# ERGO-Code/ipx

Measured on AMD Instinct MI355X. Metric: kkt_solves_per_sec, higher is better.
Workload: dtype f64

## Files before the change

ipx_amd/csrc/internal.hpp:

```cpp
#pragma once

#include <hip/hip_runtime.h>

#include <cstdint>
#include <cstdio>
#include <cstdlib>
#include <algorithm>
#include <cstring>
#include <memory>
#include <stdexcept>
#include <string>
#include <type_traits>
#include <vector>

#include "../../include/ipx_kkt_hip.h"

namespace ipxk {

struct Error : std::runtime_error {
    int code;
    Error(int c, const std::string& what) : std::runtime_error(what), code(c) {}
};

void set_last_error(const std::string& msg);
// ... 69 lines not shown
constexpr int kLongSeg = 2048;
constexpr int kMaxWorkgroups = 1024;
constexpr int kMaxPartials = 2048;
constexpr int kMaxRT = 8;

struct GatherView {
    int nrows, ncols;
    int P, G, RT, Q;
    int RWrows;
    const int* step_ptr;
    const int* wg_chunk_ptr;
    const int* chunk_start;
    const int* chunk_info;
    const int* chunk_step;
    const unsigned char* counts;
    const int* idx;
    const double* val;
    const unsigned char* row_long;
    int nseg;
    const int* seg_p0;
    const int* seg_p1;
    const int* lidx;
    const double* lval;
    int nlong;
    const int* long_row;
    const int* long_slot;
    double* long_partials;
    unsigned long long* stamps;
    int masked;
};

constexpr int kSlicedRows = 1024;
constexpr int kSlicedMaxTile = 7680;

struct SlicedView {
    int nrows, nrows_pad, nslices, nrb;
    int R;
    const unsigned* tile_ptr;
    const unsigned char* cnt;
    const int* idx;
    const double* val;
    double* partial;
    const unsigned char* row_long;
    int masked;
};

struct SlicedMatrix {
    bool built = false;
    int nslices = 0, nrb = 0, nrows_pad = 0, max_tile = 0, R = kSlicedRows;
    double dominant_fraction = 1.0;
    DevBuf<unsigned> tile_ptr;
    DevBuf<unsigned char> cnt;
    DevBuf<int> idx;
    DevBuf<double> val, partial;
};

constexpr int kSortedThreads = 256;
constexpr int kSortedMaxSub = 8192;
constexpr int kSortedOffBits = 18;
struct SortedView {
    int nrows, nrows_pad, nslices, nsub, nrb, RB, slice_elems;
    const int* xmin;
    const unsigned char* row_long;
    const unsigned* sub_ptr;
    const unsigned char* cnt;
    const unsigned* pack;
    const double* val;
    double* partial;
};
struct SortedMatrix {
    bool built = false;
    int nslices = 0, nsub = 0, nrb = 0, RB = 0, nrows_pad = 0, max_sub = 0, slice_elems = 0;
    DevBuf<unsigned> sub_ptr, pack;
    DevBuf<unsigned char> cnt;
    DevBuf<double> val, partial;
    bool fused = false;
    DevBuf<int> xmin;
};

constexpr int kAccThreads = 512;
constexpr int kAccPerThread = 4;
constexpr int kAccBatch = kAccThreads * kAccPerThread;
constexpr int kAccMaxRows = 16384;
struct AccView {
    int nrows, nrows_pad, nslices, nrb, RB, slice_elems;
    const int* xmin;
    const unsigned* tile_batch;
    const unsigned* bptr;
    const unsigned* pack;
    const double* val;
    double* partial;
};
struct AccMatrix {
    bool built = false;
    int nslices = 0, nrb = 0, RB = 0, nrows_pad = 0, slice_elems = 0;
    int64_t nbatches = 0, deferred = 0;
    DevBuf<unsigned> tile_batch, bptr, pack;
    DevBuf<double> val, partial;
    bool fused = false;
    DevBuf<int> xmin;
};

struct LayoutScratch;

struct GatherMatrix {
    int nrows = 0, ncols = 0;
    int64_t nnz = 0;
    int P = 1, G = 1, RT = 1, Q = 1, RWrows = kBlock;
    DevBuf<int> step_ptr, idx, wg_chunk_ptr, chunk_start, chunk_info, chunk_step;
    DevBuf<unsigned char> counts, row_long;
    DevBuf<double> val;
    int nseg = 0, nlong = 0;
    DevBuf<int> seg_p0, seg_p1, lidx, long_row, long_slot;
    DevBuf<double> lval, long_partials;
    DevBuf<unsigned long long> stamps;
    int tune_level = 2;
    bool keep_plain = false;
    std::vector<int> h_plain_ptr;
    DevBuf<int> plain_idx;
    DevBuf<double> plain_val;

    void build(int64_t nrows_, int64_t ncols_, const ipxint* hptr, const ipxint* hidx,
               const double* hval, hipStream_t s);
    bool build_device(LayoutScratch& S, int64_t nrows_, int64_t ncols_, int64_t nnz_, const int* dptr, const int* didx,
                      const double* dval, hipStream_t s);
    bool build_device_local(LayoutScratch& S, int64_t nrows_, int64_t ncols_, int64_t nnz_, const int* dptr, const int* didx,
                            const double* dval, double share, hipStream_t s);
    void set_geometry(int64_t nrows_, int64_t ncols_);
    SlicedMatrix sliced;
    bool use_sliced = false;
    SortedMatrix sorted;
    bool use_sorted = false;
    void build_sorted(const ipxint* hptr, const ipxint* hidx, const double* hval, hipStream_t s);
    AccMatrix acc;
    bool use_acc = false;
    float tuned_us_acc = 0.f;
    void build_acc(const ipxint* hptr, const ipxint* hidx, const double* hval, hipStream_t s);
    void build_acc_fused(const ipxint* hptr, const ipxint* hidx, const double* hval, hipStream_t s);
    AccMatrix accf;
    bool use_acc_fused = false;
    float tuned_us_acc_fused = 0.f;
    AccView acc_fused_view() const;
    AccView acc_view() const;
    const int* csr_ptr = nullptr;
    const int* csr_idx = nullptr;
    const double* csr_val = nullptr;
    bool use_plain = false;
    float tuned_us_plain = 0.f;
    int plain_grid() const { return (int)std::min<int64_t>(kMaxPartials, std::max<int64_t>(1, ((int64_t)nrows * 8 + kBlock - 1) / kBlock)); }
    void build_sorted_fused(const ipxint* hptr, const ipxint* hidx, const double* hval, hipStream_t s);
    bool use_sorted_fused = false;
    float tuned_us_sorted_fused = 0.f;
    int sorted_fused_grid() const {
        static const int cap = [] { const char* e = getenv("IPXK_SF_GRID"); return e && atoi(e) > 0 ? std::min(atoi(e), kMaxPartials) : kMaxPartials; }();
        return std::min(sorted.nrb, cap);
    }
    SortedView sorted_view() const;
    float tuned_us_phased = 0.f, tuned_us_sliced = 0.f, tuned_us_fused = 0.f, tuned_us_sorted = 0.f;
    void build_sliced(const ipxint* hptr, const ipxint* hidx, const double* hval, hipStream_t s, int ns_request);
    SlicedView sliced_view(int which = 0) const;
    int fused_grid() const { return std::min(sliced.nrb, kMaxPartials); }
    int combine_grid() const { return (int)std::min<int64_t>(1024, std::max<int64_t>(1, ((int64_t)nrows + kBlock - 1) / kBlock)); }

    GatherView view(bool masked = false) const;
    int grid() const { return G; }
    DevBuf<double> valM, lvalM;
// ... 40 lines not shown
```

ipx_amd/csrc/layout_device.hip:

```cpp
#include <rocprim/device/device_radix_sort.hpp>
#include <rocprim/device/device_scan.hpp>

#include <chrono>
#include <memory>

#include "context.hpp"

namespace ipxk {

namespace {

using u64 = unsigned long long;
#define IPXK_GS(i, n) for (int64_t i = (int64_t)blockIdx.x * blockDim.x + threadIdx.x; i < (n); i += (int64_t)gridDim.x * blockDim.x)

int gridn(int64_t n) { return (int)std::min<int64_t>(8192, std::max<int64_t>(1, (n + kBlock - 1) / kBlock)); }
int bits_for(u64 maxval) { int b = 1; while (b < 64 && (maxval >> b) != 0) b++; return b; }

__global__ void narrow_kernel(int64_t nz, const ipxint* __restrict__ in, int* __restrict__ out, int limit, int* bad) {
    IPXK_GS(p, nz) {
        const ipxint v = in[p];
        if (v < 0 || v >= limit) *bad = 1;
        out[p] = (int)v;
    }
}
__global__ void rowof_kernel(int nrows, const int* __restrict__ ptr, int* __restrict__ rowof, unsigned* __restrict__ pos) {
    IPXK_GS(r, nrows)
        for (int p = ptr[r]; p < ptr[r + 1]; p++) { rowof[p] = (int)r; if (pos) pos[p] = (unsigned)p; }
}
__global__ void gather_transposed_kernel(int64_t nz, const unsigned* __restrict__ perm, const int* __restrict__ colof,
                                         const double* __restrict__ Ax, int* __restrict__ Ti, double* __restrict__ Tx) {
    IPXK_GS(t, nz) {
        const unsigned p = perm[t];
        Ti[t] = colof[p];
        Tx[t] = Ax[p];
    }
}
template <class K>
__global__ void lower_bounds_kernel(int64_t count, int64_t nz, const K* __restrict__ sorted, u64 stride, int shift, unsigned* __restrict__ out) {
    IPXK_GS(t, count) {
        const u64 want = (u64)t * stride;
        int64_t lo = 0, hi = nz;
        while (lo < hi) { const int64_t mid = (lo + hi) >> 1; if (((u64)sorted[mid] >> shift) < want) lo = mid + 1; else hi = mid; }
        out[t] = (unsigned)lo;
    }
}
__global__ void row_pointers_kernel(int64_t m, int64_t nz, const unsigned* __restrict__ sorted_rows, int* __restrict__ Tp) {
    IPXK_GS(i, m + 1) {
        int64_t lo = 0, hi = nz;
        while (lo < hi) { const int64_t mid = (lo + hi) >> 1; if (sorted_rows[mid] < (unsigned)i) lo = mid + 1; else hi = mid; }
        Tp[i] = (int)lo;
    }
}
__global__ void max_len_kernel(int nrows, const int* __restrict__ ptr, int* out) {
    int best = 0;
    IPXK_GS(r, nrows) best = max(best, ptr[r + 1] - ptr[r]);
#pragma unroll
    for (int d = 32; d >= 1; d >>= 1) best = max(best, __shfl_xor(best, d, 64));
    if ((threadIdx.x & 63) == 0 && best > 0) atomicMax(out, best);
}
__global__ void row_extent_kernel(int n, const int* __restrict__ rows, const int* __restrict__ ptr, int* __restrict__ ext) {
    IPXK_GS(l, n) { ext[2 * l] = ptr[rows[l]]; ext[2 * l + 1] = ptr[rows[l] + 1]; }
}
__global__ void sliced_keys_kernel(int nrows, const int* __restrict__ ptr, const int* __restrict__ idx, int R, int ns, int slice,
                                   unsigned* __restrict__ key, unsigned* __restrict__ pos) {
    IPXK_GS(r, nrows) {
        const unsigned base = (unsigned)(r / R) * (unsigned)ns, rr = (unsigned)(r % R);
        for (int p = ptr[r]; p < ptr[r + 1]; p++) {
            key[p] = (base + (unsigned)(idx[p] / slice)) * (unsigned)R + rr;
            pos[p] = (unsigned)p;
        }
    }
}
__global__ void sorted_keys1_kernel(int nrows, const int* __restrict__ ptr, const int* __restrict__ idx, int RB, int ns, int nsub, int slice,
                                    int half, unsigned* __restrict__ key, unsigned* __restrict__ pos) {
    IPXK_GS(r, nrows) {
        const unsigned tile0 = (unsigned)(r / RB) * (unsigned)ns, rr = (unsigned)(r % RB);
        for (int p = ptr[r]; p < ptr[r + 1]; p++) {
            const int sl = idx[p] / slice, off = idx[p] - sl * slice;
            const unsigned sub = (tile0 + (unsigned)sl) * (unsigned)nsub + (unsigned)min(off / half, nsub - 1);
            key[p] = sub * (unsigned)RB + rr;
            pos[p] = (unsigned)p;
        }
// ... 490 lines not shown
        out.tile_ptr.ensure((size_t)ntiles + 1);
        hipLaunchKernelGGL(lower_bounds_kernel<unsigned>, dim3(gridn(ntiles + 1)), dim3(kBlock), 0, s, ntiles + 1, nnz, S.k2.get(), (u64)R, 0,
                           out.tile_ptr.get());
        IPXK_HIP(hipMemsetAsync(S.stats.get(), 0, 8 * sizeof(int), s));
        hipLaunchKernelGGL(tile_stats_kernel, dim3(gridn(nrb)), dim3(kBlock), 0, s, nrb, ns, out.tile_ptr.get(), S.stats.get());
        IPXK_HIP(hipMemcpyAsync(h, S.stats.get(), sizeof h, hipMemcpyDeviceToHost, s));
        IPXK_HIP(hipStreamSynchronize(s));
        if (h[0] <= kSlicedMaxTile) break;
    }
    u64 dom = 0;
    memcpy(&dom, h + 2, sizeof dom);
    out.dominant_fraction = (double)(int64_t)dom / (double)nnz;
    const size_t nslots = (size_t)ntiles * R;
    out.cnt.ensure(nslots); out.idx.ensure(nz); out.val.ensure(nz);
    IPXK_HIP(hipMemsetAsync(out.cnt.get(), 0, nslots, s));
    IPXK_HIP(hipMemsetAsync(S.stats.get(), 0, 8 * sizeof(int), s));
    hipLaunchKernelGGL(run_counts_kernel, dim3(gridn(nnz)), dim3(kBlock), 0, s, nnz, S.k2.get(), out.cnt.get(), S.stats.get());
    hipLaunchKernelGGL(gather_entries_kernel, dim3(gridn(nnz)), dim3(kBlock), 0, s, nnz, S.v2.get(), didx, dval, out.idx.get(), out.val.get());
    int over = 0;
    IPXK_HIP(hipMemcpyAsync(&over, S.stats.get(), sizeof(int), hipMemcpyDeviceToHost, s));
    IPXK_HIP(hipStreamSynchronize(s));
    IPXK_HIP(hipGetLastError());
    if (over) { out = SlicedMatrix(); return false; }
    out.R = R; out.nslices = ns; out.nrb = nrb; out.nrows_pad = nrb * R; out.max_tile = h[0];
    out.partial.resize(ns > 1 ? (size_t)ns * out.nrows_pad : 1);
    out.built = true;
    return true;
}

bool device_build_sorted(LayoutScratch& S, SortedMatrix& out, const SlicedMatrix& sliced, int nrows, int ncols, int64_t nnz, const int* dptr,
                         const int* didx, const double* dval, hipStream_t s) {
    out = SortedMatrix();
    if (!sliced.built || sliced.nslices < 2 || nnz == 0) return false;
    const int ns = sliced.nslices;
    const int64_t slice = (((int64_t)ncols + ns - 1) / ns + 15) / 16 * 16;
    if (slice > (int64_t(1) << kSortedOffBits)) return false;
    static const int nsub_env = [] { const char* e = getenv("IPXK_SORTED_NSUB"); return e && atoi(e) > 0 ? std::min(atoi(e), 16) : 2; }();
    const int nsub = nsub_env;
    const int64_t half = (slice / nsub + 15) / 16 * 16;
    const size_t nz = (size_t)nnz;
    S.k1.ensure(nz); S.k2.ensure(nz); S.v1.ensure(nz); S.v2.ensure(nz); S.v3.ensure(nz); S.v4.ensure(nz); S.q1.ensure(nz); S.q2.ensure(nz);
    S.stats.ensure(8);
    int RB = 32 * kSortedThreads, nrb = 0, max_sub = 0;
    int64_t nsubs = 0;
    for (;; RB /= 2) {
        if (RB < 4 * kSortedThreads) return false;
        nrb = (nrows + RB - 1) / RB;
        nsubs = (int64_t)nrb * ns * nsub;
        if ((u64)nsubs * (u64)RB >= (u64(1) << 32)) return false;
        hipLaunchKernelGGL(sorted_keys1_kernel, dim3(gridn(nrows)), dim3(kBlock), 0, s, nrows, dptr, didx, RB, ns, nsub, (int)slice, (int)half,
                           S.k1.get(), S.v1.get());
        sort_pairs<unsigned>(S.T, S.k1.get(), S.k2.get(), S.v1.get(), S.v2.get(), nz, bits_for((u64)nsubs * (u64)RB - 1), s);
        out.sub_ptr.ensure((size_t)nsubs + 1);
        hipLaunchKernelGGL(lower_bounds_kernel<unsigned>, dim3(gridn(nsubs + 1)), dim3(kBlock), 0, s, nsubs + 1, nnz, S.k2.get(), (u64)RB, 0,
                           out.sub_ptr.get());
        IPXK_HIP(hipMemsetAsync(S.stats.get(), 0, 8 * sizeof(int), s));
        hipLaunchKernelGGL(max_range_kernel, dim3(gridn(nsubs)), dim3(kBlock), 0, s, nsubs, out.sub_ptr.get(), S.stats.get());
        IPXK_HIP(hipMemcpyAsync(&max_sub, S.stats.get(), sizeof(int), hipMemcpyDeviceToHost, s));
        IPXK_HIP(hipStreamSynchronize(s));
        if (max_sub <= kSortedMaxSub) break;
    }
    const size_t nslots = (size_t)nsubs * RB;
    out.cnt.ensure(nslots); out.pack.ensure(nz); out.val.ensure(nz);
    IPXK_HIP(hipMemsetAsync(out.cnt.get(), 0, nslots, s));
    IPXK_HIP(hipMemsetAsync(S.stats.get(), 0, 8 * sizeof(int), s));
    hipLaunchKernelGGL(run_counts_kernel, dim3(gridn(nnz)), dim3(kBlock), 0, s, nnz, S.k2.get(), out.cnt.get(), S.stats.get());
    hipLaunchKernelGGL(sorted_keys2_kernel, dim3(gridn(nnz)), dim3(kBlock), 0, s, nnz, S.k2.get(), S.v2.get(), didx, RB, ns, nsub, (int)slice,
                       S.q1.get(), S.v3.get());
    sort_pairs<u64>(S.T, S.q1.get(), S.q2.get(), S.v3.get(), S.v4.get(), nz, kSortedOffBits + bits_for((u64)nsubs - 1), s);
    hipLaunchKernelGGL(sorted_fill_kernel, dim3(gridn(nnz)), dim3(kBlock), 0, s, nnz, S.q2.get(), S.v4.get(), S.v2.get(), out.sub_ptr.get(), dval,
                       out.pack.get(), out.val.get());
    int over = 0;
    IPXK_HIP(hipMemcpyAsync(&over, S.stats.get(), sizeof(int), hipMemcpyDeviceToHost, s));
    IPXK_HIP(hipStreamSynchronize(s));
    IPXK_HIP(hipGetLastError());
    if (over) { out = SortedMatrix(); return false; }
    out.nslices = ns; out.nsub = nsub; out.nrb = nrb; out.RB = RB; out.nrows_pad = nrb * RB;
    out.max_sub = max_sub; out.slice_elems = (int)slice;
    out.partial.resize((size_t)ns * out.nrows_pad);
    out.built = true;
    return true;
}

int acc_rows_per_block(int nrows, int ns) {
    static const int cap = [] { const char* e = getenv("IPXK_ACC_ROWS"); return e && atoi(e) >= 1024 ? std::min(atoi(e), kAccMaxRows) : kAccMaxRows; }();
    int RB = cap;
    while (RB > 1024 && ((int64_t)nrows + RB - 1) / RB * (int64_t)ns < 256) RB /= 2;
    return RB;
}

bool device_build_acc(LayoutScratch& S, AccMatrix& out, const SlicedMatrix& sliced, int nrows, int ncols, int64_t nnz, const int* dptr,
                      const int* didx, const double* dval, hipStream_t s) {
    out = AccMatrix();
    if (!sliced.built || sliced.nslices < 2 || nnz == 0) return false;
    const int ns = sliced.nslices;
    const int64_t slice = (((int64_t)ncols + ns - 1) / ns + 15) / 16 * 16;
    if (slice > (int64_t(1) << kSortedOffBits)) return false;
    const int RB = acc_rows_per_block(nrows, ns);
    const int nrb = (nrows + RB - 1) / RB;
    const int64_t ntiles = (int64_t)nrb * ns;
    const size_t nz = (size_t)nnz;
    S.q1.ensure(nz); S.q2.ensure(nz); S.v1.ensure(nz); S.v2.ensure(nz); S.v3.ensure(nz); S.v4.ensure(nz); S.k1.ensure(nz); S.k2.ensure(nz);
    S.stats.ensure(8);
    DevBuf<int> rowof(nz);
    DevBuf<unsigned> tile_ptr((size_t)ntiles + 1), nbatch((size_t)ntiles + 1), bstart(nz);
    hipLaunchKernelGGL(acc_keys_kernel, dim3(gridn(nrows)), dim3(kBlock), 0, s, nrows, dptr, didx, RB, ns, (int)slice, S.q1.get(), S.v1.get(), rowof.get());
    sort_pairs<u64>(S.T, S.q1.get(), S.q2.get(), S.v1.get(), S.v2.get(), nz, kSortedOffBits + bits_for((u64)std::max<int64_t>(ntiles, 2) - 1), s);
    hipLaunchKernelGGL(lower_bounds_kernel<u64>, dim3(gridn(ntiles + 1)), dim3(kBlock), 0, s, ntiles + 1, nnz, S.q2.get(), (u64)1, kSortedOffBits,
                       tile_ptr.get());
    unsigned* word = S.k1.get();
    hipLaunchKernelGGL(acc_words_kernel, dim3(gridn(nnz)), dim3(kBlock), 0, s, nnz, S.q2.get(), S.v2.get(), rowof.get(), RB, word);
    IPXK_HIP(hipMemsetAsync(S.stats.get(), 0, 8 * sizeof(int), s));
    const size_t lds = (size_t)RB * 2 * sizeof(unsigned);
    IPXK_HIP(hipFuncSetAttribute(reinterpret_cast<const void*>(acc_batch_kernel), hipFuncAttributeMaxDynamicSharedMemorySize,
                                 (int)(kAccMaxRows * 2 * sizeof(unsigned))));
    hipLaunchKernelGGL(acc_batch_kernel, dim3((unsigned)ntiles), dim3(64), lds, s, RB, tile_ptr.get(), word, S.k2.get(), S.v3.get(), S.v4.get(),
                       bstart.get(), nbatch.get(), reinterpret_cast<u64*>(S.stats.get()));
    out.tile_batch.ensure((size_t)ntiles + 1);
    hipLaunchKernelGGL(scan_u32_kernel, dim3(1), dim3(1024), 0, s, (int)ntiles, nbatch.get(), out.tile_batch.get());
    unsigned nb_total = 0;
    u64 ndef = 0;
    IPXK_HIP(hipMemcpyAsync(&nb_total, out.tile_batch.get() + ntiles, sizeof(unsigned), hipMemcpyDeviceToHost, s));
    IPXK_HIP(hipMemcpyAsync(&ndef, S.stats.get(), sizeof(u64), hipMemcpyDeviceToHost, s));
    IPXK_HIP(hipStreamSynchronize(s));
    out.bptr.ensure((size_t)nb_total + 1); out.pack.ensure(nz); out.val.ensure(nz);
    hipLaunchKernelGGL(acc_bptr_kernel, dim3((unsigned)ntiles), dim3(64), 0, s, (int)ntiles, tile_ptr.get(), out.tile_batch.get(), bstart.get(),
                       (unsigned)nnz, out.bptr.get());
    hipLaunchKernelGGL(acc_scatter_kernel, dim3(gridn(nnz)), dim3(kBlock), 0, s, nnz, S.k2.get(), word, S.v2.get(), dval, out.pack.get(),
                       out.val.get());
    IPXK_HIP(hipStreamSynchronize(s));
    IPXK_HIP(hipGetLastError());
    out.nslices = ns; out.nrb = nrb; out.RB = RB; out.nrows_pad = nrb * RB; out.slice_elems = (int)slice;
    out.nbatches = nb_total; out.deferred = (int64_t)ndef;
    out.partial.resize((size_t)ns * out.nrows_pad);
    out.built = true;
    return true;
}

bool device_build_sorted_fused(LayoutScratch& S, SortedMatrix& out, int nrows, int ncols, int64_t nnz, const int* dptr, const int* didx,
                               const double* dval, hipStream_t s) {
    out = SortedMatrix();
    if (nrows == 0 || nnz == 0 || ncols == 0) return false;
    static const int cap = [] { const char* e = getenv("IPXK_SF_MAXSUB"); return e && atoi(e) >= 256 ? std::min(atoi(e), kSortedMaxSub) : kSortedMaxSub; }();
    const size_t nz = (size_t)nnz;
    S.q1.ensure(nz); S.q2.ensure(nz); S.v1.ensure(nz); S.v2.ensure(nz); S.stats.ensure(8);
    DevBuf<int> lo, hi;
    int RB = 32 * kSortedThreads, nrb = 0, h[4] = {0, 0, 0, 0};
    for (;; RB /= 2) {
        if (RB < kSortedThreads) return false;
        nrb = (nrows + RB - 1) / RB;
        if (RB > kSortedThreads && nrb < 1024) continue;
        lo.ensure((size_t)nrb); hi.ensure((size_t)nrb);
        out.cnt.ensure((size_t)nrb * RB);
        IPXK_HIP(hipMemsetAsync(lo.get(), 0x7f, (size_t)nrb * sizeof(int), s));
        IPXK_HIP(hipMemsetAsync(hi.get(), 0xff, (size_t)nrb * sizeof(int), s));
        IPXK_HIP(hipMemsetAsync(out.cnt.get(), 0, (size_t)nrb * RB, s));
        IPXK_HIP(hipMemsetAsync(S.stats.get(), 0, 8 * sizeof(int), s));
        hipLaunchKernelGGL(tile_window_kernel, dim3(gridn(nrows)), dim3(kBlock), 0, s, nrows, dptr, didx, RB, lo.get(), hi.get(), out.cnt.get(), S.stats.get() + 2);
        hipLaunchKernelGGL(tile_window_stats_kernel, dim3(gridn(nrb)), dim3(kBlock), 0, s, nrb, nrows, RB, dptr, lo.get(), hi.get(), S.stats.get());
        IPXK_HIP(hipMemcpyAsync(h, S.stats.get(), sizeof h, hipMemcpyDeviceToHost, s));
        IPXK_HIP(hipStreamSynchronize(s));
        if (h[2]) { out = SortedMatrix(); return false; }
        if (h[1] <= cap) break;
    }
    if (h[0] >= (1 << kSortedOffBits)) { out = SortedMatrix(); return false; }
    hipLaunchKernelGGL(fused_keys_kernel, dim3(gridn(nrows)), dim3(kBlock), 0, s, nrows, dptr, didx, RB, lo.get(), S.q1.get(), S.v1.get(), (int*)nullptr);
    sort_pairs<u64>(S.T, S.q1.get(), S.q2.get(), S.v1.get(), S.v2.get(), nz, kSortedOffBits + bits_for((u64)std::max(nrb, 2) - 1), s);
    out.sub_ptr.ensure((size_t)nrb + 1); out.pack.ensure(nz); out.val.ensure(nz); out.xmin.ensure((size_t)nrb);
// ... 314 lines not shown
```

ipx_amd/csrc/nmatrix.hip:

```cpp
#include <rocprim/device/device_radix_sort.hpp>
#include <rocprim/device/device_scan.hpp>

#include "context.hpp"
#include "spmv_kernels.hpp"
#include "trisolve.hpp"

namespace ipxk {

namespace {

using u64 = unsigned long long;
constexpr int kTileShift = 42, kRowShift = 32;
#define IPXK_GS(i, n) for (int64_t i = (int64_t)blockIdx.x * blockDim.x + threadIdx.x; i < (n); i += (int64_t)gridDim.x * blockDim.x)

int gridn(int64_t n) { return (int)std::min<int64_t>(4096, std::max<int64_t>(1, (n + kBlock - 1) / kBlock)); }

__global__ void nm_keep_kernel(int n, const double* __restrict__ W, const int* __restrict__ Ap, int* __restrict__ keep, int* __restrict__ len) {
    IPXK_GS(j, n) {
        const int k = W[j] != 0.0 ? 1 : 0;
        keep[j] = k;
        len[j] = k ? Ap[j + 1] - Ap[j] : 0;
    }
}
__global__ void nm_colof_kernel(int n, const int* __restrict__ keep, const int* __restrict__ newidx, int* __restrict__ colof,
// ... 221 lines not shown
        const int nN = last[0] + last[1];
        const int64_t nzN = (int64_t)last[2] + last[3];
        if (nN < 1 || nzN < 1) return false;
        N.nN = nN;
        N.colof.ensure((size_t)nN);
        hipLaunchKernelGGL(nm_colof_kernel, dim3(gridn(n)), dim3(kBlock), 0, s, n, N.keep.get(), N.newidx.get(), N.colof.get(), N.newidx.get());
        N.keys.ensure((size_t)c->nnz); N.keys2.ensure((size_t)c->nnz);
        int64_t slice1 = 0, slice2 = 0;
        const int ns1 = slices_for(m, &slice1), ns2 = slices_for(nN, &slice2);
        N.P1 = SlicedMatrix(); N.P2 = SlicedMatrix();
        bool ok = false;
        for (int R = kSlicedRows; R >= kBlock && !ok; R /= 2) {
            hipLaunchKernelGGL(nm_keys_p1_kernel, dim3(gridn(n)), dim3(kBlock), 0, s, n, c->pl_Ap.get(), c->pl_Ai.get(), N.newidx.get(), N.off.get(), R,
                               ns1, (int)slice1, N.keys.get());
            sort_u64(N.T, N.keys.get(), N.keys2.get(), (size_t)nzN, s);
            ok = finish_layout(N, N.P1, nN, R, ns1, nzN, N.keys2.get(), c->pl_Ai.get(), c->pl_Ax.get(), nullptr, s);
        }
        if (!ok) return false;
        ok = false;
        for (int R = kSlicedRows; R >= kBlock && !ok; R /= 2) {
            hipLaunchKernelGGL(nm_keys_p2_kernel, dim3(gridn(m)), dim3(kBlock), 0, s, m, c->pl_Tp.get(), c->pl_Ti.get(), N.newidx.get(), R, ns2, (int)slice2,
                               N.keys.get());
            sort_u64(N.T, N.keys.get(), N.keys2.get(), (size_t)c->nnz, s);
            ok = finish_layout(N, N.P2, m, R, ns2, nzN, N.keys2.get(), c->pl_Ti.get(), c->pl_Tx.get(), N.newidx.get(), s);
        }
        if (!ok) return false;
        N.A1 = AccMatrix(); N.A2 = AccMatrix();
        if (!(getenv("IPXK_SPMV_ACC") && getenv("IPXK_SPMV_ACC")[0] == '0') && ns1 > 1 && ns2 > 1) {
            std::unique_ptr<LayoutScratch, void (*)(LayoutScratch*)> LS(new_layout_scratch(), free_layout_scratch);
            const size_t nzn = (size_t)nzN;
            N.cptr.ensure((size_t)std::max(nN, m) + 1); N.cidx.ensure(nzn); N.cval.ensure(nzn);
            hipLaunchKernelGGL(nm_csr1_kernel, dim3(gridn(nN)), dim3(kBlock), 0, s, nN, nzN, N.colof.get(), N.off.get(), c->pl_Ap.get(), c->pl_Ai.get(),
                               c->pl_Ax.get(), N.cptr.get(), N.cidx.get(), N.cval.get());
            AccMatrix a1, a2;
            const bool ok1 = device_build_acc(*LS, a1, N.P1, nN, m, nzN, N.cptr.get(), N.cidx.get(), N.cval.get(), s);
            N.cnt32.ensure((size_t)m + 1);
            hipLaunchKernelGGL(nm_csr2_count_kernel, dim3(gridn(m)), dim3(kBlock), 0, s, m, c->pl_Tp.get(), c->pl_Ti.get(), N.newidx.get(), N.cnt32.get());
            scan_int(N.T, N.cnt32.get(), N.cptr.get(), (size_t)m, s);
            hipLaunchKernelGGL(nm_csr2_fill_kernel, dim3(gridn(m)), dim3(kBlock), 0, s, m, nzN, c->pl_Tp.get(), c->pl_Ti.get(), c->pl_Tx.get(),
                               N.newidx.get(), N.cptr.get(), N.cidx.get(), N.cval.get());
            const bool ok2 = device_build_acc(*LS, a2, N.P2, m, nN, nzN, N.cptr.get(), N.cidx.get(), N.cval.get(), s);
            if (ok1 && ok2) { N.A1 = std::move(a1); N.A2 = std::move(a2); }
        }
        N.wN.ensure((size_t)nN); N.tN.ensure((size_t)nN);
        N.kept_hash = hsh;
        N.keep_built.ensure((size_t)n);
        IPXK_HIP(hipMemcpyAsync(N.keep_built.get(), N.keep.get(), (size_t)n * sizeof(int), hipMemcpyDeviceToDevice, s));
        N.valid = true;
        if (getenv("IPXK_VERBOSE"))
            fprintf(stderr, "ipxk: N built on the device: %d of %d structural columns, %lld entries; N'u tiles %d x %d (rows %d), N t tiles %d x %d (rows %d)\n",
                    nN, n, (long long)nzN, N.P1.nrb, N.P1.nslices, N.P1.R, N.P2.nrb, N.P2.nslices, N.P2.R);
    }
    hipLaunchKernelGGL(nm_weights_kernel, dim3(gridn(N.nN)), dim3(kBlock), 0, s, N.nN, N.colof.get(), W, N.wN.get());
    IPXK_HIP(hipGetLastError());
    return true;
}

void nmatrix_invalidate(Context* c) { if (c->nmat) c->nmat->valid = false; }

static SlicedView view_of(const SlicedMatrix& P, int nrows) {
    SlicedView V;
    V.nrows = nrows; V.nrows_pad = P.nrows_pad; V.nslices = P.nslices; V.nrb = P.nrb; V.R = P.R;
    V.tile_ptr = P.tile_ptr.get(); V.cnt = P.cnt.get(); V.idx = P.idx.get(); V.val = P.val.get(); V.partial = P.partial.get();
    V.row_long = nullptr; V.masked = 0;
    return V;
}
template <class Epi>
static void launch_tiles(const SlicedMatrix& P, int nrows, const double* x, const Epi& epi, const int* done, hipStream_t s) {
    const SlicedView V = view_of(P, nrows);
    const size_t lds = (size_t)(P.max_tile + P.max_tile / 32 + 1) * sizeof(double);
    const dim3 grid(V.nrb * V.nslices), block(kBlock);
    if (V.R == kBlock * 4) hipLaunchKernelGGL((spmv_sliced_tile_kernel<Epi, 4, false, false>), grid, block, lds, s, V, x, epi, (double*)nullptr, done);
    else if (V.R == kBlock * 2) hipLaunchKernelGGL((spmv_sliced_tile_kernel<Epi, 2, false, false>), grid, block, lds, s, V, x, epi, (double*)nullptr, done);
    else hipLaunchKernelGGL((spmv_sliced_tile_kernel<Epi, 1, false, false>), grid, block, lds, s, V, x, epi, (double*)nullptr, done);
    const int cg = (int)std::min<int64_t>(1024, std::max<int64_t>(1, ((int64_t)nrows + kBlock - 1) / kBlock));
    hipLaunchKernelGGL(spmv_sliced_combine_kernel<Epi>, dim3(cg), dim3(kBlock), 0, s, V, epi, (double*)nullptr, done);
}

template <class Epi>
static void launch_acc(const AccMatrix& A, const SlicedMatrix& P, int nrows, const double* x, const Epi& epi, const int* done, hipStream_t s) {
    AccView W;
    W.nrows = nrows; W.nrows_pad = A.nrows_pad; W.nslices = A.nslices; W.nrb = A.nrb; W.RB = A.RB; W.slice_elems = A.slice_elems;
    W.tile_batch = A.tile_batch.get(); W.bptr = A.bptr.get(); W.pack = A.pack.get(); W.val = A.val.get(); W.partial = A.partial.get();
    static bool lds_attr_set = false;
    if (!lds_attr_set) {
        IPXK_HIP(hipFuncSetAttribute(reinterpret_cast<const void*>(spmv_acc_tile_kernel<Epi>), hipFuncAttributeMaxDynamicSharedMemorySize,
                                     (int)(kAccMaxRows * sizeof(double))));
        lds_attr_set = true;
    }
    hipLaunchKernelGGL((spmv_acc_tile_kernel<Epi>), dim3(W.nrb * W.nslices), dim3(kAccThreads), (size_t)W.RB * sizeof(double), s, W, x, done);
    SlicedView V = view_of(P, nrows);
    V.nrows_pad = A.nrows_pad; V.partial = A.partial.get();
    const int cg = (int)std::min<int64_t>(1024, std::max<int64_t>(1, ((int64_t)nrows + kBlock - 1) / kBlock));
    hipLaunchKernelGGL(spmv_sliced_combine_kernel<Epi>, dim3(cg), dim3(kBlock), 0, s, V, epi, (double*)nullptr, done);
}

void nmatrix_apply(Context* c, const double* WI, const double* u, double* work, const int* done) {
    NMatrix& N = *c->nmat;
    hipStream_t s = c->stream;
    EpiScale e1{{}, N.wN.get(), N.tN.get()};
    EpiNormalRows e2{{}, WI, u, work};
    if (N.A1.built && N.A2.built) {
        launch_acc(N.A1, N.P1, N.nN, u, e1, done, s);
        launch_acc(N.A2, N.P2, (int)c->m, N.tN.get(), e2, done, s);
        return;
    }
    launch_tiles(N.P1, N.nN, u, e1, done, s);
    launch_tiles(N.P2, (int)c->m, N.tN.get(), e2, done, s);
}

}
```

ipx_amd/csrc/spmv_kernels.hpp:

```cpp
#pragma once

#include "device_utils.hpp"
#include "internal.hpp"

namespace ipxk {

constexpr int kLdsDoubles = kChunkNnz + kChunkNnz / 32;

__device__ __forceinline__ int lds_slot(int q) { return q + (q >> 5); }

struct ProdMul {
    static __device__ __forceinline__ double prod(double xg, double v) { return xg * v; }
};
struct ProdSquareWeighted {
    static __device__ __forceinline__ double prod(double xg, double v) { return (v * xg) * v; }
};

struct EpiScale : ProdMul {
    const double* w; double* out;
    static constexpr bool kNeg = false;
    __device__ __forceinline__ double init(int) const { return 0.0; }
    __device__ __forceinline__ void finish(int r, double acc, double&) const {
        out[r] = w ? acc * w[r] : acc;
    }
// ... 535 lines not shown
            p += cq;
        }
        __syncthreads();
    }
    if (dot_partials) {
        double d = dotpart;
#pragma unroll
        for (int o = 32; o > 0; o >>= 1) d += __shfl_down(d, o, 64);
        if (lane == 0) red[wave] = d;
        __syncthreads();
        if (tid == 0) {
            double t = 0.0;
            for (int w = 0; w < kSortedThreads / 64; w++) t += red[w];
            dot_partials[blockIdx.x] = t;
        }
    }
}

template <class Prod>
__global__ __launch_bounds__(kAccThreads) void spmv_acc_tile_kernel(AccView M, const double* __restrict__ x, const int* done) {
    if (done && *done) return;
    extern __shared__ double ac_sum[];
    constexpr int U = kAccPerThread, T = kAccThreads;
    const int tid = threadIdx.x;
    const int tile = blockIdx.x, s = tile % M.nslices, rb = tile / M.nslices;
    const double* __restrict__ xs = x + (size_t)s * M.slice_elems;
    const unsigned b0 = M.tile_batch[tile];
    const int nb = (int)(M.tile_batch[tile + 1] - b0);
    auto first = [&](int k) -> unsigned { return M.bptr[b0 + min(k, nb)]; };
    constexpr int NE = 6;
    unsigned e[NE];
#pragma unroll
    for (int i = 0; i < NE; i++) e[i] = first(i);
    unsigned pk[3][U];
    double v[3][U], xg[2][U];
    auto stream = [&](unsigned (&pkb)[U], double (&vb)[U], unsigned e0, unsigned e1) {
        const int ne = (int)(e1 - e0);
        if (ne <= 0) return;
#pragma unroll
        for (int u = 0; u < U; u++) {
            const int i = min(u * T + tid, ne - 1);
            pkb[u] = __builtin_nontemporal_load(M.pack + e0 + i);
            vb[u] = __builtin_nontemporal_load(M.val + e0 + i);
        }
    };
    auto gather = [&](double (&xgb)[U], const unsigned (&pkb)[U]) {
#pragma unroll
        for (int u = 0; u < U; u++) xgb[u] = xs[pkb[u] & ((1u << kSortedOffBits) - 1u)];
    };
#pragma unroll
    for (int d = 0; d < 3; d++) {
#pragma unroll
        for (int u = 0; u < U; u++) { pk[d][u] = 0u; v[d][u] = 0.0; }
        stream(pk[d], v[d], e[d], e[d + 1]);
    }
    for (int r = tid; r < M.RB; r += T) ac_sum[r] = 0.0;
    if (nb > 0) gather(xg[0], pk[0]);
    for (int k0 = 0; k0 < nb; k0 += 6) {
#pragma unroll
        for (int d = 0; d < 6; d++) {
            const int k = k0 + d;
            if (k < nb) {
                const int ne = (int)(e[1] - e[0]);
                if (k + 1 < nb) gather(xg[(d + 1) & 1], pk[(d + 1) % 3]);
                const unsigned enew = first(k + NE);
                __syncthreads();
#pragma unroll
                for (int u = 0; u < U; u++)
                    if (u * T + tid < ne)
                        __hip_atomic_fetch_add(ac_sum + (pk[d % 3][u] >> kSortedOffBits), Prod::prod(xg[d & 1][u], v[d % 3][u]), __ATOMIC_RELAXED,
                                               __HIP_MEMORY_SCOPE_WORKGROUP);
                stream(pk[d % 3], v[d % 3], e[3], e[4]);
#pragma unroll
                for (int i = 0; i + 1 < NE; i++) e[i] = e[i + 1];
                e[NE - 1] = enew;
            }
        }
    }
    __syncthreads();
    double* dst = M.partial + (size_t)s * M.nrows_pad + (size_t)rb * M.RB;
    for (int r = 2 * tid; r < M.RB; r += 2 * T) reinterpret_cast<double2*>(dst + r)[0] = make_double2(ac_sum[r], ac_sum[r + 1]);
}

template <class Epi>
__global__ __launch_bounds__(kBlock) void spmv_rowgroup_kernel(int nrows, const int* __restrict__ ptr, const int* __restrict__ idx,
                                                               const double* __restrict__ val, const unsigned char* __restrict__ row_long,
                                                               const double* __restrict__ x, Epi epi, double* dot_partials, const int* done) {
    if (done && *done) return;
    __shared__ double red[kBlock / 64 + 1];
    const int lane8 = threadIdx.x & 7, lane = threadIdx.x & 63, g0 = lane & ~7;
    double dotpart = 0.0;
    const int ngroups = (gridDim.x * kBlock) >> 3;
    for (int r = (blockIdx.x * kBlock + threadIdx.x) >> 3; r < nrows; r += ngroups) {
        const bool live = !(row_long && row_long[r]);
        const int p0 = ptr[r], p1 = live ? ptr[r + 1] : p0;
        double acc = lane8 == 0 ? epi.init(r) : 0.0;
        for (int p = p0; p < p1; p += 8) {
            const int q = p + lane8;
            const double prod = q < p1 ? Epi::prod(x[idx[q]], val[q]) : 0.0;
#pragma unroll
            for (int k = 0; k < 8; k++) {
                const double t = __shfl(prod, g0 + k, 64);
                if (p + k < p1) acc = Epi::kNeg ? acc - t : acc + t;
            }
        }
        if (live && lane8 == 0) epi.finish(r, acc, dotpart);
    }
    if (dot_partials) {
        const double d = block_reduce<SumOp>(dotpart, red);
        if (threadIdx.x == 0) dot_partials[blockIdx.x] = d;
    }
}

template <class Epi>
__global__ __launch_bounds__(kAccThreads) void spmv_acc_fused_kernel(AccView M, const double* __restrict__ x, Epi epi, double* dot_partials,
                                                                     const int* done) {
    if (done && *done) return;
    extern __shared__ double ac_sum[];
    __shared__ double red[kAccThreads / 64];
    constexpr int U = kAccPerThread, T = kAccThreads;
    const int tid = threadIdx.x;
    const int tile = blockIdx.x;
    const double* __restrict__ xs = x + M.xmin[tile];
    const unsigned b0 = M.tile_batch[tile];
    const int nb = (int)(M.tile_batch[tile + 1] - b0);
    auto first = [&](int k) -> unsigned { return M.bptr[b0 + min(k, nb)]; };
    constexpr int NE = 6;
    unsigned e[NE];
#pragma unroll
    for (int i = 0; i < NE; i++) e[i] = first(i);
    unsigned pk[3][U];
    double v[3][U], xg[2][U];
    auto stream = [&](unsigned (&pkb)[U], double (&vb)[U], unsigned e0, unsigned e1) {
        const int ne = (int)(e1 - e0);
        if (ne <= 0) return;
#pragma unroll
        for (int u = 0; u < U; u++) {
            const int i = min(u * T + tid, ne - 1);
            pkb[u] = __builtin_nontemporal_load(M.pack + e0 + i);
            vb[u] = __builtin_nontemporal_load(M.val + e0 + i);
        }
    };
    auto gather = [&](double (&xgb)[U], const unsigned (&pkb)[U]) {
#pragma unroll
        for (int u = 0; u < U; u++) xgb[u] = xs[pkb[u] & ((1u << kSortedOffBits) - 1u)];
    };
#pragma unroll
    for (int d = 0; d < 3; d++) {
#pragma unroll
        for (int u = 0; u < U; u++) { pk[d][u] = 0u; v[d][u] = 0.0; }
        stream(pk[d], v[d], e[d], e[d + 1]);
    }
    const int r0 = tile * M.RB;
    for (int r = tid; r < M.RB; r += T) ac_sum[r] = r0 + r < M.nrows ? epi.init(r0 + r) : 0.0;
    if (nb > 0) gather(xg[0], pk[0]);
    for (int k0 = 0; k0 < nb; k0 += 6) {
#pragma unroll
        for (int d = 0; d < 6; d++) {
            const int k = k0 + d;
            if (k < nb) {
                const int ne = (int)(e[1] - e[0]);
                if (k + 1 < nb) gather(xg[(d + 1) & 1], pk[(d + 1) % 3]);
                const unsigned enew = first(k + NE);
                __syncthreads();
#pragma unroll
                for (int u = 0; u < U; u++)
                    if (u * T + tid < ne) {
                        const double p = Epi::prod(xg[d & 1][u], v[d % 3][u]);
                        __hip_atomic_fetch_add(ac_sum + (pk[d % 3][u] >> kSortedOffBits), Epi::kNeg ? -p : p, __ATOMIC_RELAXED, __HIP_MEMORY_SCOPE_WORKGROUP);
                    }
                stream(pk[d % 3], v[d % 3], e[3], e[4]);
#pragma unroll
                for (int i = 0; i + 1 < NE; i++) e[i] = e[i + 1];
                e[NE - 1] = enew;
            }
        }
    }
    __syncthreads();
    double dotpart = 0.0;
    for (int r = tid; r < M.RB; r += T)
        if (r0 + r < M.nrows) epi.finish(r0 + r, ac_sum[r], dotpart);
    if (dot_partials) {
#pragma unroll
        for (int o = 32; o > 0; o >>= 1) dotpart += __shfl_down(dotpart, o, 64);
        if ((tid & 63) == 0) red[tid >> 6] = dotpart;
        __syncthreads();
        if (tid == 0) {
            double t = 0.0;
            for (int w = 0; w < T / 64; w++) t += red[w];
            dot_partials[tile] = t;
        }
    }
}

template <class Epi>
__global__ __launch_bounds__(kBlock) void spmv_sliced_combine_kernel(SlicedView M, Epi epi, double* dot_partials,
                                                                     const int* done) {
    if (done && *done) return;
    __shared__ double red[kBlock / 64 + 1];
    double dotpart = 0.0;
    for (int r = blockIdx.x * kBlock + threadIdx.x; r < M.nrows; r += gridDim.x * kBlock) {
        if (M.row_long && M.row_long[r]) continue;
        double acc = epi.init(r);
        for (int s = 0; s < M.nslices; s++) {
            const double t = __builtin_nontemporal_load(M.partial + (size_t)s * M.nrows_pad + r);
            acc = Epi::kNeg ? acc - t : acc + t;
        }
        epi.finish(r, acc, dotpart);
    }
    if (dot_partials) {
        const double d = block_reduce<SumOp>(dotpart, red);
        if (threadIdx.x == 0) dot_partials[blockIdx.x] = d;
    }
}

template <class Epi, bool MASKED = false, bool COMPACT = false>
inline void launch_spmv_sliced(const GatherMatrix& M, const double* x, const Epi& epi, double* dot_partials,
                               const int* done, hipStream_t s) {
    static_assert(!(MASKED && COMPACT), "the compacted copy needs no mask");
    if (M.use_acc && !MASKED && !COMPACT) {
        const AccView W = M.acc_view();
        const size_t lds = (size_t)W.RB * sizeof(double);
        static bool lds_attr_set = false;
        if (!lds_attr_set) {
            IPXK_HIP(hipFuncSetAttribute(reinterpret_cast<const void*>(spmv_acc_tile_kernel<Epi>), hipFuncAttributeMaxDynamicSharedMemorySize,
                                         (int)(kAccMaxRows * sizeof(double))));
            lds_attr_set = true;
        }
        hipLaunchKernelGGL((spmv_acc_tile_kernel<Epi>), dim3(W.nrb * W.nslices), dim3(kAccThreads), lds, s, W, x, done);
        SlicedView C = M.sliced_view(0);
        C.nrows_pad = W.nrows_pad; C.partial = W.partial;
        hipLaunchKernelGGL(spmv_sliced_combine_kernel<Epi>, dim3(M.combine_grid()), dim3(kBlock), 0, s, C, epi, dot_partials, done);
        if (M.nlong > 0) {
            const GatherView G = M.view(false);
            hipLaunchKernelGGL(spmv_long_kernel<Epi>, dim3(M.nseg), dim3(kBlock), 0, s, G, x, done);
            hipLaunchKernelGGL(spmv_long_fixup_kernel<Epi>, dim3(1), dim3(kBlock), 0, s, G, epi, dot_partials, M.combine_grid(), done);
        }
        return;
    }
    const SlicedView V = M.sliced_view(COMPACT ? 2 : MASKED ? 1 : 0);
    const size_t lds = (size_t)(M.sliced.max_tile + M.sliced.max_tile / 32 + 1) * sizeof(double);
    const dim3 grid(V.nrb * V.nslices), block(kBlock);
    if (V.nslices == 1) {
        const dim3 fgrid(M.fused_grid());
        if (V.R == kBlock * 4) hipLaunchKernelGGL((spmv_sliced_tile_kernel<Epi, 4, true, MASKED>), fgrid, block, lds, s, V, x, epi, dot_partials, done);
        else if (V.R == kBlock * 2) hipLaunchKernelGGL((spmv_sliced_tile_kernel<Epi, 2, true, MASKED>), fgrid, block, lds, s, V, x, epi, dot_partials, done);
        else hipLaunchKernelGGL((spmv_sliced_tile_kernel<Epi, 1, true, MASKED>), fgrid, block, lds, s, V, x, epi, dot_partials, done);
    } else {
        if (V.R == kBlock * 4) hipLaunchKernelGGL((spmv_sliced_tile_kernel<Epi, 4, false, MASKED>), grid, block, lds, s, V, x, epi, dot_partials, done);
        else if (V.R == kBlock * 2) hipLaunchKernelGGL((spmv_sliced_tile_kernel<Epi, 2, false, MASKED>), grid, block, lds, s, V, x, epi, dot_partials, done);
        else hipLaunchKernelGGL((spmv_sliced_tile_kernel<Epi, 1, false, MASKED>), grid, block, lds, s, V, x, epi, dot_partials, done);
        hipLaunchKernelGGL(spmv_sliced_combine_kernel<Epi>, dim3(M.combine_grid()), dim3(kBlock), 0, s, V, epi,
                           dot_partials, done);
    }
    if (M.nlong > 0) {
        const GatherView G = M.view(MASKED || COMPACT);
        hipLaunchKernelGGL(spmv_long_kernel<Epi>, dim3(M.nseg), block, 0, s, G, x, done);
        hipLaunchKernelGGL(spmv_long_fixup_kernel<Epi>, dim3(1), block, 0, s, G, epi, dot_partials,
                           V.nslices == 1 ? M.fused_grid() : M.combine_grid(), done);
    }
}

template <class Epi, bool MASKED = false>
inline int launch_spmv(const GatherMatrix& M, const double* x, const Epi& epi, double* dot_partials,
                       const int* done, hipStream_t s) {
    if (M.use_acc_fused && !MASKED) {
        const AccView W = M.acc_fused_view();
        static bool lds_attr_set = false;
        if (!lds_attr_set) {
            IPXK_HIP(hipFuncSetAttribute(reinterpret_cast<const void*>(spmv_acc_fused_kernel<Epi>), hipFuncAttributeMaxDynamicSharedMemorySize,
                                         (int)(kAccMaxRows * sizeof(double))));
            lds_attr_set = true;
        }
        hipLaunchKernelGGL((spmv_acc_fused_kernel<Epi>), dim3(W.nrb), dim3(kAccThreads), (size_t)W.RB * sizeof(double), s, W, x, epi, dot_partials, done);
        return dot_partials ? W.nrb : 0;
    }
    if (M.use_plain && !MASKED) {
        const int grid = M.plain_grid();
        hipLaunchKernelGGL(spmv_rowgroup_kernel<Epi>, dim3(grid), dim3(kBlock), 0, s, M.nrows, M.csr_ptr, M.csr_idx, M.csr_val,
                           M.nlong > 0 ? M.row_long.get() : nullptr, x, epi, dot_partials, done);
        if (M.nlong > 0) {
            const GatherView G = M.view(false);
            hipLaunchKernelGGL(spmv_long_kernel<Epi>, dim3(M.nseg), dim3(kBlock), 0, s, G, x, done);
            hipLaunchKernelGGL(spmv_long_fixup_kernel<Epi>, dim3(1), dim3(kBlock), 0, s, G, epi, dot_partials, grid, done);
        }
        return dot_partials ? grid + (M.nlong > 0 ? 1 : 0) : 0;
    }
    if (M.use_sorted_fused && !MASKED) {
        const SortedView W = M.sorted_view();
        const size_t lds = (size_t)(M.sorted.max_sub + M.sorted.max_sub / 32 + 1) * sizeof(double);
        const dim3 grid(M.sorted_fused_grid()), block(kSortedThreads);
        switch (W.RB / kSortedThreads) {
            case 32: hipLaunchKernelGGL((spmv_sorted_fused_kernel<Epi, 32>), grid, block, lds, s, W, x, epi, dot_partials, done); break;
            case 16: hipLaunchKernelGGL((spmv_sorted_fused_kernel<Epi, 16>), grid, block, lds, s, W, x, epi, dot_partials, done); break;
            case 8: hipLaunchKernelGGL((spmv_sorted_fused_kernel<Epi, 8>), grid, block, lds, s, W, x, epi, dot_partials, done); break;
            case 4: hipLaunchKernelGGL((spmv_sorted_fused_kernel<Epi, 4>), grid, block, lds, s, W, x, epi, dot_partials, done); break;
            case 2: hipLaunchKernelGGL((spmv_sorted_fused_kernel<Epi, 2>), grid, block, lds, s, W, x, epi, dot_partials, done); break;
            default: hipLaunchKernelGGL((spmv_sorted_fused_kernel<Epi, 1>), grid, block, lds, s, W, x, epi, dot_partials, done); break;
        }
        if (M.nlong > 0) {
            const GatherView G = M.view(false);
            hipLaunchKernelGGL(spmv_long_kernel<Epi>, dim3(M.nseg), dim3(kBlock), 0, s, G, x, done);
            hipLaunchKernelGGL(spmv_long_fixup_kernel<Epi>, dim3(1), dim3(kBlock), 0, s, G, epi, dot_partials, M.sorted_fused_grid(), done);
        }
        return dot_partials ? M.sorted_fused_grid() + (M.nlong > 0 ? 1 : 0) : 0;
    }
    if (M.use_sliced) {
        if (MASKED && M.compact.valid) launch_spmv_sliced<Epi, false, true>(M, x, epi, dot_partials, done, s);
        else launch_spmv_sliced<Epi, MASKED>(M, x, epi, dot_partials, done, s);
        return dot_partials ? M.num_partials() : 0;
    }
    const GatherView V = M.view(MASKED);
// ... 16 lines not shown
```

Baseline: 55.06.

## Add persistent LDS-accumulator SpMV kernel with tile-balanced row blocking

Adds a persistent-grid version of the LDS-atomic accumulation SpMV. One block per CU walks tiles with a stride, prefetches packed indices and values several batches ahead, and double-buffers the x gathers. When a tile finishes, its LDS row sums are parked in registers and written out a little at a time, so the stores overlap the next tile's work. Row-block size is also chosen so the tile count divides evenly across the persistent grid. The cost is higher register pressure and more complex synchronisation, and the partial layout now assumes RB-strided tiles, so any error in tile ordering or the parked-store logic would corrupt results.

Measured after the change: 57.31, median of 6. 4.1% higher.

```diff
diff --git a/ipx_amd/csrc/internal.hpp b/ipx_amd/csrc/internal.hpp
--- a/ipx_amd/csrc/internal.hpp
+++ b/ipx_amd/csrc/internal.hpp
@@ -175,6 +175,7 @@
 constexpr int kAccPerThread = 4;
 constexpr int kAccBatch = kAccThreads * kAccPerThread;
 constexpr int kAccMaxRows = 16384;
+int acc_persist_grid(int ns);
 struct AccView {
     int nrows, nrows_pad, nslices, nrb, RB, slice_elems;
     const int* xmin;
diff --git a/ipx_amd/csrc/layout_device.hip b/ipx_amd/csrc/layout_device.hip
--- a/ipx_amd/csrc/layout_device.hip
+++ b/ipx_amd/csrc/layout_device.hip
@@ -1,3 +1,4 @@
+#include <numeric>
 #include <rocprim/device/device_radix_sort.hpp>
 #include <rocprim/device/device_scan.hpp>
 
@@ -654,8 +655,29 @@
     return true;
 }
 
+int acc_persist_grid(int ns) {
+    static const int setting = [] { const char* e = getenv("IPXK_ACC_PERSIST"); return e ? std::max(0, atoi(e)) : 1; }();
+    if (setting == 0 || ns < 1) return 0;
+    static int cus[64] = {};
+    int dev = 0;
+    IPXK_HIP(hipGetDevice(&dev));
+    if (dev < 0 || dev >= 64) dev = 0;
+    if (cus[dev] == 0) IPXK_HIP(hipDeviceGetAttribute(&cus[dev], hipDeviceAttributeMultiprocessorCount, dev));
+    const int L = std::lcm(8, ns);
+    const int n = setting > 1 ? std::min(setting, cus[dev]) : cus[dev];
+    return std::max(L, n / L * L);
+}
+
 int acc_rows_per_block(int nrows, int ns) {
-    static const int cap = [] { const char* e = getenv("IPXK_ACC_ROWS"); return e && atoi(e) >= 1024 ? std::min(atoi(e), kAccMaxRows) : kAccMaxRows; }();
+    static const int cap = [] { const char* e = getenv("IPXK_ACC_ROWS"); return e && atoi(e) >= 1024 ? std::min(atoi(e), kAccMaxRows) & ~1 : kAccMaxRows; }();
+    static const bool balance = !(getenv("IPXK_ACC_BALANCE") && getenv("IPXK_ACC_BALANCE")[0] == '0');
+    if (const int G = balance ? acc_persist_grid(ns) : 0) {
+        const int64_t per = G / ns;
+        const int64_t nrb = (((int64_t)nrows + cap - 1) / cap + per - 1) / per * per;
+        int rb = (int)(((int64_t)nrows + nrb - 1) / nrb);
+        rb += rb & 1;
+        if (rb >= 1024 && 8 * (int64_t)rb >= 7 * (int64_t)cap) return rb;
+    }
     int RB = cap;
     while (RB > 1024 && ((int64_t)nrows + RB - 1) / RB * (int64_t)ns < 256) RB /= 2;
     return RB;
diff --git a/ipx_amd/csrc/nmatrix.hip b/ipx_amd/csrc/nmatrix.hip
--- a/ipx_amd/csrc/nmatrix.hip
+++ b/ipx_amd/csrc/nmatrix.hip
@@ -327,13 +327,7 @@
     AccView W;
     W.nrows = nrows; W.nrows_pad = A.nrows_pad; W.nslices = A.nslices; W.nrb = A.nrb; W.RB = A.RB; W.slice_elems = A.slice_elems;
     W.tile_batch = A.tile_batch.get(); W.bptr = A.bptr.get(); W.pack = A.pack.get(); W.val = A.val.get(); W.partial = A.partial.get();
-    static bool lds_attr_set = false;
-    if (!lds_attr_set) {
-        IPXK_HIP(hipFuncSetAttribute(reinterpret_cast<const void*>(spmv_acc_tile_kernel<Epi>), hipFuncAttributeMaxDynamicSharedMemorySize,
-                                     (int)(kAccMaxRows * sizeof(double))));
-        lds_attr_set = true;
-    }
-    hipLaunchKernelGGL((spmv_acc_tile_kernel<Epi>), dim3(W.nrb * W.nslices), dim3(kAccThreads), (size_t)W.RB * sizeof(double), s, W, x, done);
+    launch_acc_tiles<Epi>(W, x, done, s);
     SlicedView V = view_of(P, nrows);
     V.nrows_pad = A.nrows_pad; V.partial = A.partial.get();
     const int cg = (int)std::min<int64_t>(1024, std::max<int64_t>(1, ((int64_t)nrows + kBlock - 1) / kBlock));
diff --git a/ipx_amd/csrc/spmv_kernels.hpp b/ipx_amd/csrc/spmv_kernels.hpp
--- a/ipx_amd/csrc/spmv_kernels.hpp
+++ b/ipx_amd/csrc/spmv_kernels.hpp
@@ -641,6 +641,128 @@
     for (int r = 2 * tid; r < M.RB; r += 2 * T) reinterpret_cast<double2*>(dst + r)[0] = make_double2(ac_sum[r], ac_sum[r + 1]);
 }
 
+constexpr int kAccParkPairs = kAccMaxRows / (2 * kAccThreads);
+constexpr int kAccParkPerBatch = 2;
+template <class Prod>
+__global__ __launch_bounds__(kAccThreads) void spmv_acc_persist_kernel(AccView M, const unsigned* __restrict__ tile_batch,
+                                                                       const unsigned* __restrict__ bptr, const double* __restrict__ x,
+                                                                       const int* done) {
+    if (done && *done) return;
+    extern __shared__ double ac_sum[];
+    constexpr int U = kAccPerThread, T = kAccThreads, NP = kAccParkPairs, PB = kAccParkPerBatch;
+    static_assert(NP % PB == 0, "parked pairs per batch");
+    const int tid = threadIdx.x;
+    const int ntiles = M.nrb * M.nslices, G = gridDim.x;
+    const int s = blockIdx.x % M.nslices;
+    const double* __restrict__ xs = x + (size_t)s * M.slice_elems;
+    double* const part = M.partial + (size_t)s * M.nrows_pad;
+    struct Batch { unsigned e0, e1; int tile; };
+    int wt = blockIdx.x, wq = 0, wnb = 0;
+    unsigned wb0 = 0;
+    if (wt < ntiles) { wb0 = tile_batch[wt]; wnb = (int)(tile_batch[wt + 1] - wb0); }
+    auto next = [&]() -> Batch {
+        Batch b{0u, 0u, -1};
+        if (wt >= ntiles) return b;
+        b.tile = wt;
+        if (wnb > 0) { b.e0 = bptr[wb0 + wq]; b.e1 = bptr[wb0 + wq + 1]; }
+        if (++wq >= max(wnb, 1)) {
+            wt += G; wq = 0;
+            if (wt < ntiles) { wb0 = tile_batch[wt]; wnb = (int)(tile_batch[wt + 1] - wb0); }
+        }
+        return b;
+    };
+    constexpr int NE = 6;
+    Batch q[NE];
+#pragma unroll
+    for (int i = 0; i < NE; i++) q[i] = next();
+    unsigned pk[3][U];
+    double v[3][U], xg[2][U];
+    auto stream = [&](unsigned (&pkb)[U], double (&vb)[U], unsigned e0, unsigned e1) {
+        const int ne = (int)(e1 - e0);
+        const unsigned base = ne > 0 ? e0 : 0u;
+        const int last = max(ne - 1, 0);
+#pragma unroll
+        for (int u = 0; u < U; u++) {
+            const int i = min(u * T + tid, last);
+            pkb[u] = __builtin_nontemporal_load(M.pack + base + i);
+            vb[u] = __builtin_nontemporal_load(M.val + base + i);
+        }
+    };
+    auto gather = [&](double (&xgb)[U], const unsigned (&pkb)[U], const Batch& b) {
+        const bool live = b.e1 > b.e0;
+        const double* __restrict__ xb = live ? xs : x;
+        const unsigned mask = live ? (1u << kSortedOffBits) - 1u : 0u;
+#pragma unroll
+        for (int u = 0; u < U; u++) xgb[u] = xb[pkb[u] & mask];
+    };
+#pragma unroll
+    for (int d = 0; d < 3; d++) {
+#pragma unroll
+        for (int u = 0; u < U; u++) { pk[d][u] = 0u; v[d][u] = 0.0; }
+        stream(pk[d], v[d], q[d].e0, q[d].e1);
+    }
+    for (int r = tid; r < M.RB; r += T) ac_sum[r] = 0.0;
+    gather(xg[0], pk[0], q[0]);
+    int cur = q[0].tile;
+    double2 park[NP];
+#pragma unroll
+    for (int j = 0; j < NP; j++) park[j] = make_double2(0.0, 0.0);
+    int pleft = 0, prow = 0;
+    double* pdst = part;
+    auto store_parked = [&]() {
+#pragma unroll
+        for (int j = 0; j < PB; j++)
+            if (prow + 2 * T * j < M.RB) reinterpret_cast<double2*>(pdst + prow + 2 * T * j)[0] = park[j];
+#pragma unroll
+        for (int j = 0; j + PB < NP; j++) park[j] = park[j + PB];
+        prow += 2 * T * PB;
+        pleft--;
+    };
+    while (q[0].tile >= 0) {
+#pragma unroll
+        for (int d = 0; d < 6; d++) {
+            if (q[0].tile >= 0) {
+                const int ne = (int)(q[0].e1 - q[0].e0);
+                gather(xg[(d + 1) & 1], pk[(d + 1) % 3], q[1]);
+                __syncthreads();
+                if (q[0].tile != cur) {
+                    while (pleft > 0) store_parked();
+#pragma unroll
+                    for (int j = 0; j < NP; j++) {
+                        const int r = 2 * tid + 2 * T * j;
+                        if (r < M.RB) {
+                            park[j] = make_double2(ac_sum[r], ac_sum[r + 1]);
+                            ac_sum[r] = 0.0;
+                            ac_sum[r + 1] = 0.0;
+                        }
+                    }
+                    pdst = part + (size_t)(cur / M.nslices) * M.RB;
+                    prow = 2 * tid;
+                    pleft = NP / PB;
+                    cur = q[0].tile;
+                    __syncthreads();
+                }
+#pragma unroll
+                for (int u = 0; u < U; u++)
+                    if (u * T + tid < ne)
+                        __hip_atomic_fetch_add(ac_sum + (pk[d % 3][u] >> kSortedOffBits), Prod::prod(xg[d & 1][u], v[d % 3][u]), __ATOMIC_RELAXED,
+                                               __HIP_MEMORY_SCOPE_WORKGROUP);
+                stream(pk[d % 3], v[d % 3], q[3].e0, q[3].e1);
+                if (pleft > 0) store_parked();
+#pragma unroll
+                for (int i = 0; i + 1 < NE; i++) q[i] = q[i + 1];
+                q[NE - 1] = next();
+            }
+        }
+    }
+    __syncthreads();
+    while (pleft > 0) store_parked();
+    if (cur >= 0) {
+        double* dst = part + (size_t)(cur / M.nslices) * M.RB;
+        for (int r = 2 * tid; r < M.RB; r += 2 * T) reinterpret_cast<double2*>(dst + r)[0] = make_double2(ac_sum[r], ac_sum[r + 1]);
+    }
+}
+
 template <class Epi>
 __global__ __launch_bounds__(kBlock) void spmv_rowgroup_kernel(int nrows, const int* __restrict__ ptr, const int* __restrict__ idx,
                                                                const double* __restrict__ val, const unsigned char* __restrict__ row_long,
@@ -773,20 +895,30 @@
     }
 }
 
+template <class Prod>
+inline void launch_acc_tiles(const AccView& W, const double* x, const int* done, hipStream_t s) {
+    static bool lds_attr_set = false;
+    if (!lds_attr_set) {
+        IPXK_HIP(hipFuncSetAttribute(reinterpret_cast<const void*>(spmv_acc_tile_kernel<Prod>), hipFuncAttributeMaxDynamicSharedMemorySize,
+                                     (int)(kAccMaxRows * sizeof(double))));
+        IPXK_HIP(hipFuncSetAttribute(reinterpret_cast<const void*>(spmv_acc_persist_kernel<Prod>), hipFuncAttributeMaxDynamicSharedMemorySize,
+                                     (int)(kAccMaxRows * sizeof(double))));
+        lds_attr_set = true;
+    }
+    const size_t lds = (size_t)W.RB * sizeof(double);
+    const int ntiles = W.nrb * W.nslices, G = acc_persist_grid(W.nslices);
+    if (G > 0) hipLaunchKernelGGL((spmv_acc_persist_kernel<Prod>), dim3(std::min(G, ntiles)), dim3(kAccThreads), lds, s, W, W.tile_batch, W.bptr,
+                                  x, done);
+    else hipLaunchKernelGGL((spmv_acc_tile_kernel<Prod>), dim3(ntiles), dim3(kAccThreads), lds, s, W, x, done);
+}
+
 template <class Epi, bool MASKED = false, bool COMPACT = false>
 inline void launch_spmv_sliced(const GatherMatrix& M, const double* x, const Epi& epi, double* dot_partials,
                                const int* done, hipStream_t s) {
     static_assert(!(MASKED && COMPACT), "the compacted copy needs no mask");
     if (M.use_acc && !MASKED && !COMPACT) {
         const AccView W = M.acc_view();
-        const size_t lds = (size_t)W.RB * sizeof(double);
-        static bool lds_attr_set = false;
-        if (!lds_attr_set) {
-            IPXK_HIP(hipFuncSetAttribute(reinterpret_cast<const void*>(spmv_acc_tile_kernel<Epi>), hipFuncAttributeMaxDynamicSharedMemorySize,
-                                         (int)(kAccMaxRows * sizeof(double))));
-            lds_attr_set = true;
-        }
-        hipLaunchKernelGGL((spmv_acc_tile_kernel<Epi>), dim3(W.nrb * W.nslices), dim3(kAccThreads), lds, s, W, x, done);
+        launch_acc_tiles<Epi>(W, x, done, s);
         SlicedView C = M.sliced_view(0);
         C.nrows_pad = W.nrows_pad; C.partial = W.partial;
         hipLaunchKernelGGL(spmv_sliced_combine_kernel<Epi>, dim3(M.combine_grid()), dim3(kBlock), 0, s, C, epi, dot_partials, done);
```
